# JoakimHaurum/TokenReduction

Measured on AMD Instinct MI355X. Metric: images/sec DeiT-S Top-K keep_rate=0.7 forward (aggregate over n_gpus; per-GPU = value/n_gpus), higher is better.
Workload: dtype bf16; 1 GPU; topk_small_patch16_224 keep_rate=0.7 reduction_loc=3,6,9 batch=256/GPU 224x224 eval forward (BASELINE.json configs[1]); global_batch=256, parallelism=dp1

## Files before the change

tokenreduction_amd/csrc/tr_mlp_fused.hip:

```cpp
#include "tr_common.h"

__device__ unsigned long long tr_mlp_clock_probe[3];

namespace {

#ifdef TR_ABLATE_NO_MFMA
#define MF_MFMA(a, b, c) ([&] { asm volatile("" ::"v"(a), "v"(b)); return c; }())
#else
#define MF_MFMA(a, b, c) __builtin_amdgcn_mfma_f32_16x16x32_bf16(a, b, c, 0, 0, 0)
#endif
__device__ __forceinline__ float mf_gelu1(float x) {
  constexpr float L2E = 1.44269504088896340736f;
  constexpr float C1 = -1.59501577f * L2E, C3 = -7.40112920e-02f * L2E, C5 = 7.03033576e-04f * L2E;
  const float xc = __builtin_amdgcn_fmed3f(x, -8.0f, 8.0f);
  const float x2 = xc * xc;
  float p = __builtin_fmaf(x2, C5, C3);
  p = __builtin_fmaf(p, x2, C1);
  const float z = p * xc;
  const float e = __builtin_amdgcn_exp2f(z) + 1.0f;
  return x * __builtin_amdgcn_rcpf(e);
}
#if defined(TR_ABLATE_NO_GELU)
__device__ __forceinline__ f32x2 mf_gelu2(f32x2 v) { return v; }
#elif defined(MF_GELU_PACKED)
// ... 3 lines not shown
  float a = mf_gelu1(v[0]), b = mf_gelu1(v[1]);
  asm volatile("" : "+v"(a), "+v"(b));
  return f32x2{a, b};
}
#endif

typedef __attribute__((ext_vector_type(4))) unsigned u32x4;
typedef __attribute__((ext_vector_type(2))) unsigned u32x2;

#ifdef MF_ABL_NO_XSTORE
#define MF_XSTORE(x) asm volatile("" ::"v"(v))
#else
#define MF_XSTORE(x) x
#endif
#ifdef MF_ABL_NO_NSTORE
#define MF_NSTORE(x) do { } while (0)
#else
#define MF_NSTORE(x) x
#endif
#ifdef TR_DIAG_STAMPS
#define MF_STAMP(k) ts_[k] = __builtin_amdgcn_s_memtime()
#define MF_STAMP_DECL unsigned long long ts_[4] = {0, 0, 0, 0}
#define MF_STAMP_DUMP(role, step)                                                                                                     \
  do {                                                                                                                                \
    if (bid == 8 && pr == 0 && lane == 0 && (step) < 64) {                                                                            \
      unsigned long long* st_ = reinterpret_cast<unsigned long long*>(reinterpret_cast<unsigned char*>(outp) + out_bytes) + ((role) * 64 + (step)) * 4; \
      st_[0] = ts_[0]; st_[1] = ts_[1]; st_[2] = ts_[2]; st_[3] = ts_[3];                                                             \
    }                                                                                                                                 \
  } while (0)
#define MF_ESTAMP(k) es_[k] = __builtin_amdgcn_s_memtime()
#define MF_ESTAMP_DECL unsigned long long es_[8] = {0, 0, 0, 0, 0, 0, 0, 0}
#define MF_ESTAMP_DUMP                                                                                                                \
  do {                                                                                                                                \
    if (bid == 8 && pr == 0 && lane == 0) {                                                                                           \
      unsigned long long* st_ = reinterpret_cast<unsigned long long*>(reinterpret_cast<unsigned char*>(outp) + out_bytes) + 60 * 4;   \
      for (int k_ = 0; k_ < 8; ++k_) st_[k_] = es_[k_];                                                                               \
    }                                                                                                                                 \
  } while (0)
#define MF_CLOCK_BEGIN const unsigned long long ck0_ = __builtin_amdgcn_s_memtime(), rt0_ = __builtin_amdgcn_s_memrealtime()
#define MF_CLOCK_END                                                                                                                  \
  do {                                                                                                                                \
    if (bid == 8 && tid == 0) {                                                                                                       \
      unsigned long long* st_ = reinterpret_cast<unsigned long long*>(reinterpret_cast<unsigned char*>(outp) + out_bytes) + 512;      \
      st_[0] = __builtin_amdgcn_s_memtime() - ck0_;                                                                                   \
      st_[1] = __builtin_amdgcn_s_memrealtime() - rt0_;                                                                               \
    }                                                                                                                                 \
  } while (0)
#elif defined(TR_DIAG_CLOCK)
#define MF_CLOCK_BEGIN const unsigned long long ck0_ = __builtin_amdgcn_s_memtime(), rt0_ = __builtin_amdgcn_s_memrealtime()
#define MF_CLOCK_END                                                                                                                  \
  do {                                                                                                                                \
    if (bid == 8 && tid == 0) {                                                                                                       \
      atomicAdd(&tr_mlp_clock_probe[0], __builtin_amdgcn_s_memtime() - ck0_);                                                         \
      atomicAdd(&tr_mlp_clock_probe[1], __builtin_amdgcn_s_memrealtime() - rt0_);                                                     \
      atomicAdd(&tr_mlp_clock_probe[2], 1ull);                                                                                        \
    }                                                                                                                                 \
  } while (0)
#define MF_STAMP(k) do { } while (0)
#define MF_STAMP_DECL do { } while (0)
#define MF_STAMP_DUMP(role, step) do { } while (0)
#define MF_ESTAMP(k) do { } while (0)
#define MF_ESTAMP_DECL do { } while (0)
#define MF_ESTAMP_DUMP do { } while (0)
#else
#define MF_CLOCK_BEGIN do { } while (0)
#define MF_CLOCK_END do { } while (0)
#define MF_STAMP(k) do { } while (0)
#define MF_STAMP_DECL do { } while (0)
#define MF_STAMP_DUMP(role, step) do { } while (0)
#define MF_ESTAMP(k) do { } while (0)
#define MF_ESTAMP_DECL do { } while (0)
#define MF_ESTAMP_DUMP do { } while (0)
#endif

constexpr int MF_D = 384;
constexpr int MF_KS = MF_D / 32;
constexpr int MF_NI = MF_D / 16;
constexpr int MF_W1FR = 2 * MF_KS;
constexpr int MF_FR = MF_W1FR + MF_NI;
constexpr int MF_ENTRY = MF_FR * 1024;
constexpr int MF_NSLOT = 3;
constexpr int MF_HBUF = 2048;
constexpr int MF_LDS = MF_NSLOT * MF_ENTRY + 4 * 2 * MF_HBUF;
constexpr int MF_ROWS = 128;
#ifndef MF_PQ
#define MF_PQ 0
#endif
#ifndef MF_DMA_BURST
#define MF_DMA_SPREAD 1
#endif
constexpr int MF_PPW = (MF_PQ + 3) / 4;
[[maybe_unused]] constexpr int MF_CPW = (12 - MF_PQ + 4) / 5;

__device__ __forceinline__ void mf_piece(const unsigned char* sbase, unsigned voff, unsigned lds_dst) {
#ifndef TR_ABLATE_NO_DMA
  asm volatile(
      "s_mov_b32 m0, %[ld]\n\t"
      "s_nop 0\n\t"
      "global_load_lds_dwordx4 %[o], %[b]"
      :
      : [o] "v"(voff), [b] "s"(sbase), [ld] "s"(lds_dst)
      : "memory", "m0");
#endif
}

template <int IMM>
__device__ __forceinline__ bf16x8 mf_load_x(const uint16_t* sbase, unsigned voff) {
  bf16x8 v;
  asm volatile("global_load_dwordx4 %0, %1, %2 offset:%3" : "=v"(v) : "v"(voff), "s"(sbase), "i"(IMM) : "memory");
  return v;
}
template <int IMM>
__device__ __forceinline__ void mf_reload_x(bf16x8& v, const uint16_t* sbase, unsigned voff) {
  asm volatile("global_load_dwordx4 %0, %1, %2 offset:%3" : "+v"(v) : "v"(voff), "s"(sbase), "i"(IMM) : "memory");
}
template <int IMM>
__device__ __forceinline__ f32x4 mf_load_f4(const float* sbase, unsigned voff) {
  f32x4 v;
  asm volatile("global_load_dwordx4 %0, %1, %2 offset:%3" : "=v"(v) : "v"(voff), "s"(sbase), "i"(IMM) : "memory");
  return v;
}

#define MF_TIE_X(x)                                                                                                                   \
  "+v"(x[0]), "+v"(x[1]), "+v"(x[2]), "+v"(x[3]), "+v"(x[4]), "+v"(x[5]), "+v"(x[6]), "+v"(x[7]), "+v"(x[8]), "+v"(x[9]), "+v"(x[10]), \
      "+v"(x[11])

__global__ __launch_bounds__(256) void mlp_pack_kernel(const uint16_t* __restrict__ W1, const uint16_t* __restrict__ W2, const float* __restrict__ b2,
                                                       u32x4* __restrict__ pk, int D, int Hd) {
  const int ks_n = D / 32, ni = D / 16, fr = 2 * ks_n + ni;
  const int g = blockIdx.x * 4 + (threadIdx.x >> 6);
  const int lane = threadIdx.x & 63;
  const int s = g / fr, f = g % fr;
  if (s >= Hd / 32) {
    const int e = g - (Hd / 32) * fr;
    if (e < 2 * ni) pk[(size_t)g * 64 + lane] = *reinterpret_cast<const u32x4*>(b2 + 16 * (e >> 1) + 4 * (lane >> 4));
    return;
  }
  const int r = lane & 15, q = lane >> 4;
  const uint16_t* src;
  if (f < 2 * ks_n) {
#ifdef MF_P32
    const int rho = lane & 31, kq = lane >> 5;
    const int hh = 8 * (((rho >> 2) & 1) + 2 * (rho >> 4)) + 4 * ((rho >> 3) & 1) + (rho & 3);
    src = W1 + (size_t)(32 * s + hh) * D + 16 * f + 8 * kq;
#else
    const int t2 = f / ks_n, ks = f % ks_n;
    src = W1 + (size_t)(32 * s + 8 * (r >> 2) + 4 * t2 + (r & 3)) * D + 32 * ks + 8 * q;
#endif
  } else {
    const int i = f - 2 * ks_n;
    src = W2 + (size_t)(16 * i + r) * Hd + 32 * s + 8 * q;
  }
  pk[(size_t)g * 64 + lane] = *reinterpret_cast<const u32x4*>(src);
}

struct MfSeq {
  int head_len, head_blk;
  int full0, fstride, nfull;
  int tail_s0, tail_blk;
};
struct MfCur {
  int seg, s;
};
__device__ __forceinline__ MfCur mf_first(const MfSeq& q, int NS) {
  if (q.head_len > 0) return MfCur{-1, 0};
  if (q.nfull > 0) return MfCur{0, 0};
// ... 17 lines not shown
constexpr unsigned MF_SK_ERR_MAGIC = 0x4d46534bu;

struct MfResid {
  float* x;
  const float* b2;
  const float* g;
  const float* b;
  float eps;
};

struct MfNorm {
  const float* x;
  const uint16_t* d;
  const float* g;
  const float* b;
  float eps;
};

template <bool RL, bool NP>
__global__ __launch_bounds__(512, 2) void mlp_fused_kernel(const uint16_t* __restrict__ xn, const unsigned char* __restrict__ pk,
                                                           const float* __restrict__ b1,
                                                           uint16_t* __restrict__ outp, unsigned char* __restrict__ scratch, int M, int NS,
                                                           unsigned out_bytes, int poll_max, int cset, const MfResid rl, const MfNorm nm) {
  __shared__ __attribute__((aligned(16))) unsigned char smem[MF_LDS];
  const int tid = threadIdx.x, lane = tid & 63;
  const int wave = __builtin_amdgcn_readfirstlane(tid >> 6);
  const int pr = wave & 3;
#ifdef MF_XCD_RANGES
  const int G = gridDim.x;
  const int bid = (G % 8 == 0 && G > 8) ? ((int)blockIdx.x & 7) * (G >> 3) + ((int)blockIdx.x >> 3) : (int)blockIdx.x;
#else
  const int G = gridDim.x, bid = blockIdx.x;
#endif
  const int nblk = (M + MF_ROWS - 1) / MF_ROWS;
  if (bid >= nblk) return;
  MfSeq q;
  int T;
  const bool streamk = scratch != nullptr && nblk > G;
  if (!streamk) {
    q = MfSeq{0, 0, bid, G, (nblk - bid + G - 1) / G, NS, 0};
    T = q.nfull * NS;
  } else {
    const long long U = (long long)nblk * NS;
    const int u0 = (int)(U * bid / G), u1 = (int)(U * (bid + 1) / G);
    const int b_first = u0 / NS, s0 = u0 - b_first * NS;
    const int b_end = u1 / NS, s1 = u1 - b_end * NS;
    const int f0 = s0 > 0 ? b_first + 1 : b_first;
    q = MfSeq{s1, b_end, f0, 1, b_end - f0, s0 > 0 ? s0 : NS, b_first};
    T = u1 - u0;
  }
  q.head_len = __builtin_amdgcn_readfirstlane(q.head_len); q.head_blk = __builtin_amdgcn_readfirstlane(q.head_blk);
  q.full0 = __builtin_amdgcn_readfirstlane(q.full0); q.fstride = __builtin_amdgcn_readfirstlane(q.fstride);
  q.nfull = __builtin_amdgcn_readfirstlane(q.nfull); q.tail_s0 = __builtin_amdgcn_readfirstlane(q.tail_s0);
  q.tail_blk = __builtin_amdgcn_readfirstlane(q.tail_blk);
  T = __builtin_amdgcn_readfirstlane(T);
  const unsigned lds0 = (unsigned)(uintptr_t)(__attribute__((address_space(3))) unsigned char*)smem;
  const unsigned lane16 = (unsigned)lane * 16u;
  const int frow = lane & 15, fq = lane >> 4;
  unsigned char* const hb = smem + MF_NSLOT * MF_ENTRY + pr * (2 * MF_HBUF);

  MfCur ld_cur = mf_first(q, NS);
  int ld_e = 0, ld_w1 = ld_cur.s, ld_w2 = ld_cur.s, ld_w2n = ld_cur.s, ld_slot = 0;
  auto issue_piece_q = [&](int q) __attribute__((always_inline)) {
    const int f = (wave < 4 ? 0 : 4 * MF_PQ) + pr + 4 * q;
    const int step = (f < MF_W1FR) ? ld_w1 : ld_w2;
    mf_piece(pk + (size_t)step * MF_ENTRY + f * 1024, lane16, lds0 + ld_slot * MF_ENTRY + f * 1024);
  };
  auto issue_all = [&]() __attribute__((always_inline)) {
    if (wave < 4) {
#pragma unroll
      for (int q = 0; q < MF_PQ; ++q) issue_piece_q(q);
    } else {
#pragma unroll
      for (int q = 0; q < 12 - MF_PQ; ++q) issue_piece_q(q);
    }
  };
  auto advance_entry = [&]() __attribute__((always_inline)) {
    ++ld_e;
    ld_w2 = ld_w2n;
    ld_w2n = ld_w1;
    ld_cur = mf_next(q, ld_cur, NS);
    ld_w1 = ld_cur.s;
    ld_slot = (ld_slot + 1 == MF_NSLOT) ? 0 : ld_slot + 1;
  };

#ifdef MF_P32
  if (wave < 4) {
    typedef __attribute__((ext_vector_type(16))) float f32x16;
    const int tc = lane & 31, hg = lane >> 5;
    bf16x8 xk[2 * MF_KS];
    auto x_offset = [&](int blk) __attribute__((always_inline)) {
      const int m = blk * MF_ROWS + pr * 32 + tc;
      return ((unsigned)min(m, M - 1) * MF_D + 8u * hg) * 2u;
    };
    {
      const unsigned xo = x_offset(mf_block(q, mf_first(q, NS)));
#define MF_LX(ks) xk[ks] = mf_load_x<(ks) * 32>(xn, xo)
      MF_LX(0); MF_LX(1); MF_LX(2); MF_LX(3); MF_LX(4); MF_LX(5); MF_LX(6); MF_LX(7); MF_LX(8); MF_LX(9); MF_LX(10); MF_LX(11);
      MF_LX(12); MF_LX(13); MF_LX(14); MF_LX(15); MF_LX(16); MF_LX(17); MF_LX(18); MF_LX(19); MF_LX(20); MF_LX(21); MF_LX(22); MF_LX(23);
#undef MF_LX
    }
    const unsigned boff = (unsigned)hg * 32u;
    f32x4 bn0, bn1, bn2, bn3;
    bn0 = mf_load_f4<0>(b1 + 32 * mf_first(q, NS).s, boff);
    bn1 = mf_load_f4<16>(b1 + 32 * mf_first(q, NS).s, boff);
    bn2 = mf_load_f4<64>(b1 + 32 * mf_first(q, NS).s, boff);
    bn3 = mf_load_f4<80>(b1 + 32 * mf_first(q, NS).s, boff);
    issue_all();
    advance_entry();
    issue_all();
    advance_entry();
#define MF_TIE_XK(lo) "+v"(xk[lo]), "+v"(xk[lo + 1]), "+v"(xk[lo + 2]), "+v"(xk[lo + 3]), "+v"(xk[lo + 4]), "+v"(xk[lo + 5]), "+v"(xk[lo + 6]), "+v"(xk[lo + 7]), "+v"(xk[lo + 8]), "+v"(xk[lo + 9]), "+v"(xk[lo + 10]), "+v"(xk[lo + 11])
    asm volatile("s_waitcnt vmcnt(0)" : "+v"(bn0), "+v"(bn1), "+v"(bn2), "+v"(bn3), MF_TIE_XK(0), MF_TIE_XK(12)::"memory");
    __builtin_amdgcn_s_barrier();
    asm volatile("" ::: "memory");

    int t = 0, cslot = 0;
    f32x4 p0, p1, p2, p3;
    p0 = p1 = p2 = p3 = f32x4{0.f, 0.f, 0.f, 0.f};
    asm volatile("" : "+v"(p0), "+v"(p1), "+v"(p2), "+v"(p3));
    bf16x8 wA[4], wB[4];
#define MF_READW(buf, base, k)                                                     \
  buf[0] = *reinterpret_cast<const bf16x8*>((base) + (4 * (k)) * 1024);            \
  buf[1] = *reinterpret_cast<const bf16x8*>((base) + (4 * (k) + 1) * 1024);        \
  buf[2] = *reinterpret_cast<const bf16x8*>((base) + (4 * (k) + 2) * 1024);        \
  buf[3] = *reinterpret_cast<const bf16x8*>((base) + (4 * (k) + 3) * 1024)
    MF_READW(wA, smem + lane16, 0);
    MF_CLOCK_BEGIN;
    const unsigned hdst = (unsigned)((tc >> 4) * 1024 + ((tc & 15) + 16 * hg) * 16);
    auto p_step = [&](int sn, const bool last, int next_blk) __attribute__((always_inline)) {
      const unsigned char* slot = smem + cslot * MF_ENTRY + lane16;
      const int nslot = (cslot + 1 == MF_NSLOT) ? 0 : cslot + 1;
      const unsigned char* slot_next = smem + nslot * MF_ENTRY + lane16;
      MF_STAMP_DECL;
      MF_STAMP(0);
      f32x16 a;
#pragma unroll
      for (int e = 0; e < 4; ++e) { a[e] = bn0[e]; a[4 + e] = bn1[e]; a[8 + e] = bn2[e]; a[12 + e] = bn3[e]; }
      u32x4 h0 = {0u, 0u, 0u, 0u}, h1 = {0u, 0u, 0u, 0u};
      unsigned xo = 0;
      const bool reload = last && next_blk >= 0;
      if (reload) xo = x_offset(next_blk);
#define MF_GELU_SLICE(k)                                                                                  \
  do {                                                                                                    \
    if ((k) == 0) { const f32x2 g0 = mf_gelu2(f32x2{p0[0], p0[1]}), g1 = mf_gelu2(f32x2{p0[2], p0[3]}); h0[0] = pack_bf16x2(g0[0], g0[1]); h0[1] = pack_bf16x2(g1[0], g1[1]); asm volatile("" : "+v"(h0[0]), "+v"(h0[1])); } \
    if ((k) == 1) { const f32x2 g0 = mf_gelu2(f32x2{p1[0], p1[1]}), g1 = mf_gelu2(f32x2{p1[2], p1[3]}); h0[2] = pack_bf16x2(g0[0], g0[1]); h0[3] = pack_bf16x2(g1[0], g1[1]); asm volatile("" : "+v"(h0[2]), "+v"(h0[3])); } \
    if ((k) == 2) { const f32x2 g0 = mf_gelu2(f32x2{p2[0], p2[1]}), g1 = mf_gelu2(f32x2{p2[2], p2[3]}); h1[0] = pack_bf16x2(g0[0], g0[1]); h1[1] = pack_bf16x2(g1[0], g1[1]); asm volatile("" : "+v"(h1[0]), "+v"(h1[1])); } \
    if ((k) == 3) { const f32x2 g0 = mf_gelu2(f32x2{p3[0], p3[1]}), g1 = mf_gelu2(f32x2{p3[2], p3[3]}); h1[2] = pack_bf16x2(g0[0], g0[1]); h1[3] = pack_bf16x2(g1[0], g1[1]); asm volatile("" : "+v"(h1[2]), "+v"(h1[3])); } \
    if ((k) == 4) {                                                                                       \
      unsigned char* dst = hb + ((t - 1) & 1) * MF_HBUF + hdst;                                           \
      *reinterpret_cast<u32x4*>(dst) = h0;                                                                \
      *reinterpret_cast<u32x4*>(dst + 512) = h1;                                                          \
    }                                                                                                     \
  } while (0)
#define MF_PMFMA(cur, k)                                                                                           \
  do {                                                                                                             \
    a = __builtin_amdgcn_mfma_f32_32x32x16_bf16(cur[0], xk[4 * (k)], a, 0, 0, 0);                                  \
    a = __builtin_amdgcn_mfma_f32_32x32x16_bf16(cur[1], xk[4 * (k) + 1], a, 0, 0, 0);                              \
    a = __builtin_amdgcn_mfma_f32_32x32x16_bf16(cur[2], xk[4 * (k) + 2], a, 0, 0, 0);                              \
    a = __builtin_amdgcn_mfma_f32_32x32x16_bf16(cur[3], xk[4 * (k) + 3], a, 0, 0, 0);                              \
  } while (0)
#define MF_RX(ks) mf_reload_x<(ks) * 32>(xk[ks], xn, xo)
#define MF_PWIN(cur, nxt, k)                                                                    \
  do {                                                                                          \
    MF_READW(nxt, slot, (k) + 1);                                                               \
    __builtin_amdgcn_sched_barrier(0);                                                          \
// ... 6 lines not shown
      bn2 = mf_load_f4<64>(b1 + 32 * sn, boff);                                                 \
      bn3 = mf_load_f4<80>(b1 + 32 * sn, boff);                                                 \
    }                                                                                           \
    if (reload) { MF_RX(4 * (k)); MF_RX(4 * (k) + 1); MF_RX(4 * (k) + 2); MF_RX(4 * (k) + 3); } \
  } while (0)
      MF_PWIN(wA, wB, 0);
      MF_PWIN(wB, wA, 1);
      MF_PWIN(wA, wB, 2);
      MF_PWIN(wB, wA, 3);
      MF_PWIN(wA, wB, 4);
      if (ld_e <= T + 1) advance_entry();
      MF_STAMP(1);
      if (last) asm volatile("s_waitcnt vmcnt(0)" ::: "memory");
      asm volatile("s_waitcnt vmcnt(0)" : "+v"(bn0), "+v"(bn1), "+v"(bn2), "+v"(bn3), MF_TIE_XK(0), MF_TIE_XK(12)::"memory");
      asm volatile("s_waitcnt lgkmcnt(0)" ::: "memory");
      MF_STAMP(2);
      __builtin_amdgcn_s_barrier();
      asm volatile("" ::: "memory");
      MF_STAMP(3);
      MF_READW(wA, slot_next, 0);
      __builtin_amdgcn_sched_barrier(0);
      MF_PMFMA(wB, 5);
      __builtin_amdgcn_sched_barrier(0);
      if (reload) { MF_RX(20); MF_RX(21); MF_RX(22); MF_RX(23); }
#undef MF_PWIN
#undef MF_GELU_SLICE
#pragma unroll
      for (int e = 0; e < 4; ++e) { p0[e] = a[e]; p1[e] = a[4 + e]; p2[e] = a[8 + e]; p3[e] = a[12 + e]; }
      MF_STAMP_DUMP(0, t);
      ++t;
      cslot = nslot;
    };
    {
      MfCur cur = mf_first(q, NS);
      for (int tt = 0; tt < T; ++tt) {
        const MfCur nxt = mf_next(q, cur, NS);
        int last = __builtin_amdgcn_readfirstlane(mf_last_of_segment(q, cur, NS) ? 1 : 0);
        asm volatile("" : "+s"(last));
        p_step(nxt.s, last != 0, (last && tt + 1 < T) ? mf_block(q, nxt) : -1);
        cur = nxt;
      }
    }
    {
      const f32x2 g0 = mf_gelu2(f32x2{p0[0], p0[1]}), g1 = mf_gelu2(f32x2{p0[2], p0[3]});
      const f32x2 g2 = mf_gelu2(f32x2{p1[0], p1[1]}), g3 = mf_gelu2(f32x2{p1[2], p1[3]});
      const u32x4 h0 = {pack_bf16x2(g0[0], g0[1]), pack_bf16x2(g1[0], g1[1]), pack_bf16x2(g2[0], g2[1]), pack_bf16x2(g3[0], g3[1])};
      const f32x2 g4 = mf_gelu2(f32x2{p2[0], p2[1]}), g5 = mf_gelu2(f32x2{p2[2], p2[3]});
      const f32x2 g6 = mf_gelu2(f32x2{p3[0], p3[1]}), g7 = mf_gelu2(f32x2{p3[2], p3[3]});
      const u32x4 h1 = {pack_bf16x2(g4[0], g4[1]), pack_bf16x2(g5[0], g5[1]), pack_bf16x2(g6[0], g6[1]), pack_bf16x2(g7[0], g7[1])};
      unsigned char* dst = hb + ((t - 1) & 1) * MF_HBUF + hdst;
      *reinterpret_cast<u32x4*>(dst) = h0;
      *reinterpret_cast<u32x4*>(dst + 512) = h1;
      asm volatile("s_waitcnt vmcnt(0) lgkmcnt(0)" ::: "memory");
      __builtin_amdgcn_s_barrier();
    }
#undef MF_PMFMA
#undef MF_READW
#undef MF_RX
#undef MF_TIE_XK
    if constexpr (RL) __builtin_amdgcn_s_barrier();
    MF_CLOCK_END;
    return;
  }
#else
  if (wave < 4) {
#ifdef MF_PRIO_P
    __builtin_amdgcn_s_setprio(MF_PRIO_P);
#endif
    bf16x8 x0[MF_KS], x1[MF_KS];
    f32x4 bn0, bn1;
    const unsigned boff = (unsigned)fq * 32u;
    auto x_offsets = [&](int blk, unsigned& o0, unsigned& o1) __attribute__((always_inline)) {
      const int m = blk * MF_ROWS + pr * 32 + frow;
      o0 = ((unsigned)min(m, M - 1) * MF_D + 8u * fq) * 2u;
      o1 = ((unsigned)min(m + 16, M - 1) * MF_D + 8u * fq) * 2u;
    };
#define MF_LOAD_X(ks)                          \
  x0[ks] = mf_load_x<(ks) * 64>(xn, xo0);      \
  x1[ks] = mf_load_x<(ks) * 64>(xn, xo1)
#define MF_RELOAD_X(ks)                        \
  mf_reload_x<(ks) * 64>(x0[ks], xn, xo0);     \
  mf_reload_x<(ks) * 64>(x1[ks], xn, xo1)
    auto ln_fill = [&](int blk) __attribute__((always_inline)) {
#pragma unroll
      for (int j = 0; j < 2; ++j) {
        const int m = min(blk * MF_ROWS + pr * 32 + frow + 16 * j, M - 1);
        const float* xr = nm.x + (size_t)m * MF_D + 8 * fq;
        const uint16_t* dr = nm.d + (size_t)m * MF_D + 8 * fq;
        f32x4 v[MF_KS][2];
        u32x4 dq[2][4];
#pragma unroll
        for (int i = 0; i < 4; ++i) dq[0][i] = *reinterpret_cast<const u32x4*>(dr + 32 * i);
#pragma unroll
        for (int ks = 0; ks < MF_KS; ++ks) {
          v[ks][0] = *reinterpret_cast<const f32x4*>(xr + 32 * ks);
          v[ks][1] = *reinterpret_cast<const f32x4*>(xr + 32 * ks + 4);
        }
        __builtin_amdgcn_sched_barrier(0);
#pragma unroll
        for (int c = 0; c < 3; ++c) {
          if (c + 1 < 3) {
#pragma unroll
            for (int i = 0; i < 4; ++i) dq[(c + 1) & 1][i] = *reinterpret_cast<const u32x4*>(dr + 32 * (4 * (c + 1) + i));
          }
          __builtin_amdgcn_sched_barrier(0);
#pragma unroll
          for (int i = 0; i < 4; ++i) {
            const u32x4 dd = dq[c & 1][i];
            const int ks = 4 * c + i;
#pragma unroll
            for (int h = 0; h < 2; ++h) {
              v[ks][h][0] += __uint_as_float(dd[2 * h] << 16); v[ks][h][1] += __uint_as_float(dd[2 * h] & 0xffff0000u);
              v[ks][h][2] += __uint_as_float(dd[2 * h + 1] << 16); v[ks][h][3] += __uint_as_float(dd[2 * h + 1] & 0xffff0000u);
            }
          }
          __builtin_amdgcn_sched_barrier(0);
        }
        float sp[4][2];
#pragma unroll
        for (int ks = 0; ks < MF_KS; ++ks)
#pragma unroll
          for (int h = 0; h < 2; ++h) {
            const float t = (v[ks][h][0] + v[ks][h][1]) + (v[ks][h][2] + v[ks][h][3]);
            sp[ks & 3][h] = (ks < 4 ? 0.f : sp[ks & 3][h]) + t;
          }
        float c0 = (sp[0][0] + sp[2][0]) + (sp[1][0] + sp[3][0]), c1 = (sp[0][1] + sp[2][1]) + (sp[1][1] + sp[3][1]);
        c0 += __shfl_xor(c0, 32); c1 += __shfl_xor(c1, 32);
        c0 += __shfl_xor(c0, 16); c1 += __shfl_xor(c1, 16);
        const float mean = (c0 + c1) / (float)MF_D;
        __builtin_amdgcn_sched_barrier(0);
#pragma unroll
        for (int ks = 0; ks < MF_KS; ++ks)
#pragma unroll
          for (int h = 0; h < 2; ++h) {
            f32x4 t = v[ks][h];
            t[0] -= mean; t[1] -= mean; t[2] -= mean; t[3] -= mean;
            v[ks][h] = t;
            const float u = __builtin_fmaf(t[0], t[0], t[1] * t[1]) + __builtin_fmaf(t[2], t[2], t[3] * t[3]);
            sp[ks & 3][h] = (ks < 4 ? 0.f : sp[ks & 3][h]) + u;
          }
        c0 = (sp[0][0] + sp[2][0]) + (sp[1][0] + sp[3][0]); c1 = (sp[0][1] + sp[2][1]) + (sp[1][1] + sp[3][1]);
        c0 += __shfl_xor(c0, 32); c1 += __shfl_xor(c1, 32);
        c0 += __shfl_xor(c0, 16); c1 += __shfl_xor(c1, 16);
        const float rstd = rsqrtf((c0 + c1) / (float)MF_D + nm.eps);
        const float* gr = nm.g + 8 * fq;
        const float* br = nm.b + 8 * fq;
        f32x4 gb[2][4];
        gb[0][0] = *reinterpret_cast<const f32x4*>(gr); gb[0][1] = *reinterpret_cast<const f32x4*>(gr + 4);
        gb[0][2] = *reinterpret_cast<const f32x4*>(br); gb[0][3] = *reinterpret_cast<const f32x4*>(br + 4);
        __builtin_amdgcn_sched_barrier(0);
#pragma unroll
        for (int ks = 0; ks < MF_KS; ++ks) {
          if (ks + 1 < MF_KS) {
            gb[(ks + 1) & 1][0] = *reinterpret_cast<const f32x4*>(gr + 32 * (ks + 1)); gb[(ks + 1) & 1][1] = *reinterpret_cast<const f32x4*>(gr + 32 * (ks + 1) + 4);
            gb[(ks + 1) & 1][2] = *reinterpret_cast<const f32x4*>(br + 32 * (ks + 1)); gb[(ks + 1) & 1][3] = *reinterpret_cast<const f32x4*>(br + 32 * (ks + 1) + 4);
          }
          __builtin_amdgcn_sched_barrier(0);
          u32x4 o;
#pragma unroll
          for (int h = 0; h < 2; ++h) {
            const f32x4 gg = gb[ks & 1][h], bb = gb[ks & 1][2 + h];
            const f32x4 t = v[ks][h];
            o[2 * h] = pack_bf16x2(__builtin_fmaf(rstd * t[0], gg[0], bb[0]), __builtin_fmaf(rstd * t[1], gg[1], bb[1]));
            o[2 * h + 1] = pack_bf16x2(__builtin_fmaf(rstd * t[2], gg[2], bb[2]), __builtin_fmaf(rstd * t[3], gg[3], bb[3]));
          }
          if (j == 0) x0[ks] = __builtin_bit_cast(bf16x8, o);
          else x1[ks] = __builtin_bit_cast(bf16x8, o);
          __builtin_amdgcn_sched_barrier(0);
        }
      }
    };
    if constexpr (NP) {
      ln_fill(mf_block(q, mf_first(q, NS)));
    } else {
      unsigned xo0, xo1;
      x_offsets(mf_block(q, mf_first(q, NS)), xo0, xo1);
      MF_LOAD_X(0); MF_LOAD_X(1); MF_LOAD_X(2); MF_LOAD_X(3); MF_LOAD_X(4); MF_LOAD_X(5);
      MF_LOAD_X(6); MF_LOAD_X(7); MF_LOAD_X(8); MF_LOAD_X(9); MF_LOAD_X(10); MF_LOAD_X(11);
    }
    bn0 = mf_load_f4<0>(b1 + 32 * mf_first(q, NS).s, boff);
    bn1 = mf_load_f4<16>(b1 + 32 * mf_first(q, NS).s, boff);
    issue_all();
    advance_entry();
    issue_all();
    advance_entry();
    asm volatile("s_waitcnt vmcnt(0)" : "+v"(bn0), "+v"(bn1), MF_TIE_X(x0), MF_TIE_X(x1)::"memory");
    __builtin_amdgcn_s_barrier();
    asm volatile("" ::: "memory");

    int t = 0, cslot = 0;
    f32x4 p00, p01, p10, p11;
    p00 = p01 = p10 = p11 = f32x4{0.f, 0.f, 0.f, 0.f};
    asm volatile("" : "+v"(p00), "+v"(p01), "+v"(p10), "+v"(p11));
    bf16x8 wA[4], wB[4];
#define MF_READW(buf, base, k)                                                                  \
  buf[0] = *reinterpret_cast<const bf16x8*>((base) + (2 * (k)) * 1024);                        \
  buf[1] = *reinterpret_cast<const bf16x8*>((base) + (MF_KS + 2 * (k)) * 1024);                \
  buf[2] = *reinterpret_cast<const bf16x8*>((base) + (2 * (k) + 1) * 1024);                    \
  buf[3] = *reinterpret_cast<const bf16x8*>((base) + (MF_KS + 2 * (k) + 1) * 1024)
    MF_READW(wA, smem + lane16, 0);
    MF_CLOCK_BEGIN;
    auto p_step = [&](int sn, const bool last, int next_blk) __attribute__((always_inline)) {
      const unsigned char* slot = smem + cslot * MF_ENTRY + lane16;
      const int nslot = (cslot + 1 == MF_NSLOT) ? 0 : cslot + 1;
      const unsigned char* slot_next = smem + nslot * MF_ENTRY + lane16;
      MF_STAMP_DECL;
      MF_STAMP(0);
      f32x4 a00 = bn0, a01 = bn0, a10 = bn1, a11 = bn1;
      u32x4 h0 = {0u, 0u, 0u, 0u}, h1 = {0u, 0u, 0u, 0u};
      unsigned xo0 = 0, xo1 = 0;
      const bool reload = last && next_blk >= 0;
      if (reload) x_offsets(next_blk, xo0, xo1);
      const bool dma = ld_e <= T + 1;
#define MF_GELU_SLICE(k)                                                                                  \
  do {                                                                                                    \
    if ((k) == 0) { const f32x2 g0 = mf_gelu2(f32x2{p00[0], p00[1]}), g1 = mf_gelu2(f32x2{p00[2], p00[3]}); h0[0] = pack_bf16x2(g0[0], g0[1]); h0[1] = pack_bf16x2(g1[0], g1[1]); asm volatile("" : "+v"(h0[0]), "+v"(h0[1])); } \
    if ((k) == 1) { const f32x2 g0 = mf_gelu2(f32x2{p10[0], p10[1]}), g1 = mf_gelu2(f32x2{p10[2], p10[3]}); h0[2] = pack_bf16x2(g0[0], g0[1]); h0[3] = pack_bf16x2(g1[0], g1[1]); asm volatile("" : "+v"(h0[2]), "+v"(h0[3])); } \
    if ((k) == 2) { const f32x2 g0 = mf_gelu2(f32x2{p01[0], p01[1]}), g1 = mf_gelu2(f32x2{p01[2], p01[3]}); h1[0] = pack_bf16x2(g0[0], g0[1]); h1[1] = pack_bf16x2(g1[0], g1[1]); asm volatile("" : "+v"(h1[0]), "+v"(h1[1])); } \
    if ((k) == 3) { const f32x2 g0 = mf_gelu2(f32x2{p11[0], p11[1]}), g1 = mf_gelu2(f32x2{p11[2], p11[3]}); h1[2] = pack_bf16x2(g0[0], g0[1]); h1[3] = pack_bf16x2(g1[0], g1[1]); asm volatile("" : "+v"(h1[2]), "+v"(h1[3])); } \
    if ((k) == 4) {                                                                                       \
      unsigned char* dst = hb + ((t - 1) & 1) * MF_HBUF + lane16;                                         \
      *reinterpret_cast<u32x4*>(dst) = h0;                                                                \
      *reinterpret_cast<u32x4*>(dst + 1024) = h1;                                                         \
    }                                                                                                     \
  } while (0)
#define MF_PMFMA(cur, k)                                                                        \
  do {                                                                                          \
    a00 = MF_MFMA(cur[0], x0[2 * (k)], a00);                                                    \
    a01 = MF_MFMA(cur[0], x1[2 * (k)], a01);                                                    \
    a10 = MF_MFMA(cur[1], x0[2 * (k)], a10);                                                    \
    a11 = MF_MFMA(cur[1], x1[2 * (k)], a11);                                                    \
    a00 = MF_MFMA(cur[2], x0[2 * (k) + 1], a00);                                                \
    a01 = MF_MFMA(cur[2], x1[2 * (k) + 1], a01);                                                \
    a10 = MF_MFMA(cur[3], x0[2 * (k) + 1], a10);                                                \
    a11 = MF_MFMA(cur[3], x1[2 * (k) + 1], a11);                                                \
  } while (0)
#define MF_PWIN(cur, nxt, k)                                                                    \
  do {                                                                                          \
    MF_READW(nxt, slot, (k) + 1);                                                               \
    __builtin_amdgcn_sched_barrier(0);                                                          \
    MF_PMFMA(cur, k);                                                                           \
    MF_GELU_SLICE(k);                                                                           \
    __builtin_amdgcn_sched_barrier(0);                                                          \
    if ((k) == 0) {                                                                             \
       \
      bn0 = mf_load_f4<0>(b1 + 32 * sn, boff);                                                  \
      bn1 = mf_load_f4<16>(b1 + 32 * sn, boff);                                                 \
    }                                                                                           \
    if ((k) >= 1 && dma) {                                                                      \
      _Pragma("unroll") for (int q_ = MF_PPW * ((k) - 1); q_ < MF_PPW * (k); ++q_)              \
        if (q_ < MF_PQ) issue_piece_q(q_);                                                      \
    }                                                                                           \
    if (!NP && reload) { MF_RELOAD_X(2 * (k)); MF_RELOAD_X(2 * (k) + 1); }                      \
  } while (0)
      MF_PWIN(wA, wB, 0);
      MF_PWIN(wB, wA, 1);
      MF_PWIN(wA, wB, 2);
      MF_PWIN(wB, wA, 3);
      MF_PWIN(wA, wB, 4);
      if (dma) advance_entry();
      MF_STAMP(1);
      if (last) asm volatile("s_waitcnt vmcnt(0)" ::: "memory");
      asm volatile("s_waitcnt vmcnt(%26)" : "+v"(bn0), "+v"(bn1), MF_TIE_X(x0), MF_TIE_X(x1) : "n"(MF_PQ) : "memory");
      asm volatile("s_waitcnt lgkmcnt(0)" ::: "memory");
      MF_STAMP(2);
      __builtin_amdgcn_s_barrier();
      asm volatile("" ::: "memory");
      MF_STAMP(3);
      MF_READW(wA, slot_next, 0);
      __builtin_amdgcn_sched_barrier(0);
      MF_PMFMA(wB, 5);
      __builtin_amdgcn_sched_barrier(0);
      if constexpr (NP) {
        if (reload) {
          ln_fill(next_blk);
          MF_READW(wA, slot_next, 0);
        }
      } else {
        if (reload) { MF_RELOAD_X(10); MF_RELOAD_X(11); }
      }
#undef MF_PWIN
#undef MF_GELU_SLICE
      p00 = a00; p01 = a01; p10 = a10; p11 = a11;
      MF_STAMP_DUMP(0, t);
      ++t;
      cslot = nslot;
    };
    {
      MfCur cur = mf_first(q, NS);
      for (int tt = 0; tt < T; ++tt) {
        const MfCur nxt = mf_next(q, cur, NS);
        int last = __builtin_amdgcn_readfirstlane(mf_last_of_segment(q, cur, NS) ? 1 : 0);
        asm volatile("" : "+s"(last));
        p_step(nxt.s, last != 0, (last && tt + 1 < T) ? mf_block(q, nxt) : -1);
        cur = nxt;
      }
    }
    {
      const f32x2 g0 = mf_gelu2(f32x2{p00[0], p00[1]}), g1 = mf_gelu2(f32x2{p00[2], p00[3]});
      const f32x2 g2 = mf_gelu2(f32x2{p10[0], p10[1]}), g3 = mf_gelu2(f32x2{p10[2], p10[3]});
      const u32x4 h0 = {pack_bf16x2(g0[0], g0[1]), pack_bf16x2(g1[0], g1[1]), pack_bf16x2(g2[0], g2[1]), pack_bf16x2(g3[0], g3[1])};
      const f32x2 g4 = mf_gelu2(f32x2{p01[0], p01[1]}), g5 = mf_gelu2(f32x2{p01[2], p01[3]});
      const f32x2 g6 = mf_gelu2(f32x2{p11[0], p11[1]}), g7 = mf_gelu2(f32x2{p11[2], p11[3]});
      const u32x4 h1 = {pack_bf16x2(g4[0], g4[1]), pack_bf16x2(g5[0], g5[1]), pack_bf16x2(g6[0], g6[1]), pack_bf16x2(g7[0], g7[1])};
      unsigned char* dst = hb + ((t - 1) & 1) * MF_HBUF + lane16;
      *reinterpret_cast<u32x4*>(dst) = h0;
      *reinterpret_cast<u32x4*>(dst + 1024) = h1;
      asm volatile("s_waitcnt vmcnt(0) lgkmcnt(0)" ::: "memory");
      __builtin_amdgcn_s_barrier();
    }
#undef MF_PMFMA
#undef MF_READW
#undef MF_LOAD_X
#undef MF_RELOAD_X
    if constexpr (RL) __builtin_amdgcn_s_barrier();
    MF_CLOCK_END;
    return;
  }

#endif
#ifdef MF_PRIO_C
  __builtin_amdgcn_s_setprio(MF_PRIO_C);
#endif
  const __amdgpu_buffer_rsrc_t orsrc = __builtin_amdgcn_make_buffer_rsrc(outp, 0, (int)out_bytes, 0x00020000);
  const unsigned char* const bias_img = pk + (size_t)NS * MF_ENTRY;
  f32x4 acc[MF_NI][2];
  const __amdgpu_buffer_rsrc_t xrsrc = __builtin_amdgcn_make_buffer_rsrc(RL ? reinterpret_cast<unsigned char*>(rl.x) : const_cast<unsigned char*>(bias_img), 0,
                                                                         RL ? (int)(2u * out_bytes) : MF_NI * 2 * 1024, 0x00020000);
  auto x_row_off = [&](int blk) __attribute__((always_inline)) { return ((unsigned)(blk * MF_ROWS + pr * 32 + frow) * MF_D + 4u * fq) * 4u; };
  if constexpr (RL) {
    const unsigned vo = x_row_off(mf_block(q, mf_first(q, NS)));
#pragma unroll
    for (int i = 0; i < MF_NI; ++i)
#pragma unroll
      for (int j = 0; j < 2; ++j)
        acc[i][j] = __builtin_bit_cast(f32x4, __builtin_amdgcn_raw_buffer_load_b128(xrsrc, vo + (unsigned)(j * 16 * MF_D * 4), i * 64, 0));
  } else {
#pragma unroll
    for (int i = 0; i < MF_NI; ++i)
#pragma unroll
      for (int j = 0; j < 2; ++j)
        acc[i][j] = __builtin_bit_cast(f32x4, __builtin_amdgcn_raw_buffer_load_b128(xrsrc, lane16 + (unsigned)((i * 2 + j) * 1024), 0, 0));
  }
  issue_all();
  advance_entry();
  issue_all();
  advance_entry();
  asm volatile("s_waitcnt vmcnt(0)" ::: "memory");
  __builtin_amdgcn_s_barrier();
  asm volatile("" ::: "memory");

  int t = 0, cslot = 0;
  bf16x8 wA[4], wB[4];
  bf16x8 h0, h1;
#define MF_READW(buf, base, k)                                                     \
  buf[0] = *reinterpret_cast<const bf16x8*>((base) + (4 * (k)) * 1024);            \
  buf[1] = *reinterpret_cast<const bf16x8*>((base) + (4 * (k) + 1) * 1024);        \
  buf[2] = *reinterpret_cast<const bf16x8*>((base) + (4 * (k) + 2) * 1024);        \
  buf[3] = *reinterpret_cast<const bf16x8*>((base) + (4 * (k) + 3) * 1024)
  for (; t < 2; ++t) {
    if (ld_e <= T + 1) {
      issue_all();
      advance_entry();
    }
    cslot = (cslot + 1 == MF_NSLOT) ? 0 : cslot + 1;
    asm volatile("s_waitcnt vmcnt(%0)" ::"n"(12 - MF_PQ) : "memory");
    __builtin_amdgcn_s_barrier();
    asm volatile("" ::: "memory");
  }
  {
    const unsigned char* hsrc = hb + (t & 1) * MF_HBUF + lane16;
    h0 = *reinterpret_cast<const bf16x8*>(hsrc);
    h1 = *reinterpret_cast<const bf16x8*>(hsrc + 1024);
    MF_READW(wA, smem + cslot * MF_ENTRY + MF_W1FR * 1024 + lane16, 0);
  }
  const __amdgpu_buffer_rsrc_t sk_out = __builtin_amdgcn_make_buffer_rsrc(scratch + (size_t)bid * MF_SK_SLOT, 0, MF_SK_SLOT, 0x00020000);
  unsigned char* const sk_cnt0 = scratch + (size_t)G * MF_SK_SLOT + MF_SK_ERR + (size_t)cset * G * MF_SK_CNT;
  unsigned* const sk_cnt_out = reinterpret_cast<unsigned*>(sk_cnt0 + (size_t)bid * MF_SK_CNT);
  unsigned* const sk_cnt_in = reinterpret_cast<unsigned*>(sk_cnt0 + (size_t)(bid > 0 ? bid - 1 : 0) * MF_SK_CNT);
  bool publish_pending = false;
  auto c_step = [&](const int fin, const bool load_next, int blk, int blk_next) __attribute__((always_inline)) {
    const bool epi = fin == 1;
    const unsigned char* slot = smem + cslot * MF_ENTRY + MF_W1FR * 1024 + lane16;
    const int nslot = (cslot + 1 == MF_NSLOT) ? 0 : cslot + 1;
    const unsigned char* slot_next = smem + nslot * MF_ENTRY + MF_W1FR * 1024 + lane16;
    MF_STAMP_DECL;
    MF_STAMP(0);
    const bool dma = ld_e <= T + 1;
#define MF_CMFMA(cur, k)                                                                                           \
  _Pragma("unroll") for (int ii = 0; ii < 4; ++ii) {                                                               \
    acc[4 * (k) + ii][0] = MF_MFMA(cur[ii], h0, acc[4 * (k) + ii][0]);                                             \
    acc[4 * (k) + ii][1] = MF_MFMA(cur[ii], h1, acc[4 * (k) + ii][1]);                                             \
  }
#if defined(MF_DMA_SPREAD)
#define MF_CWIN(cur, nxt, k)                                                                                       \
  do {                                                                                                             \
    MF_READW(nxt, slot, (k) + 1);                                                                                  \
    __builtin_amdgcn_sched_barrier(0);                                                                             \
    _Pragma("unroll") for (int ii = 0; ii < 4; ++ii) {                                                             \
      acc[4 * (k) + ii][0] = MF_MFMA(cur[ii], h0, acc[4 * (k) + ii][0]);                                           \
      acc[4 * (k) + ii][1] = MF_MFMA(cur[ii], h1, acc[4 * (k) + ii][1]);                                           \
      __builtin_amdgcn_sched_barrier(0);                                                                           \
      const int hk_ = 4 * (k) + ii;                                                                                \
      if (((hk_ + 1) * (12 - MF_PQ)) / 20 > (hk_ * (12 - MF_PQ)) / 20) {                                           \
        if (dma) issue_piece_q((hk_ * (12 - MF_PQ)) / 20);                                                         \
      }                                                                                                            \
    }                                                                                                              \
  } while (0)
#else
#define MF_CWIN(cur, nxt, k)                                                                                       \
  do {                                                                                                             \
    MF_READW(nxt, slot, (k) + 1);                                                                                  \
    __builtin_amdgcn_sched_barrier(0);                                                                             \
    MF_CMFMA(cur, k);                                                                                              \
    __builtin_amdgcn_sched_barrier(0);                                                                             \
    if (dma) {                                                                                                     \
      _Pragma("unroll") for (int q_ = MF_CPW * (k); q_ < MF_CPW * ((k) + 1); ++q_)                                 \
        if (q_ < 12 - MF_PQ) issue_piece_q(q_);                                                                    \
    }                                                                                                              \
  } while (0)
#endif
    MF_CWIN(wA, wB, 0);
    MF_CWIN(wB, wA, 1);
    MF_CWIN(wA, wB, 2);
    MF_CWIN(wB, wA, 3);
    MF_CWIN(wA, wB, 4);
#undef MF_CWIN
    if (dma) advance_entry();
    MF_STAMP(1);
    if (t <= T) {
// ... 442 lines not shown
```

Baseline: 105,900 images/s.

## Split first-block LayerNorm between producer and consumer waves via LDS hand-over

For the fused-norm prologue, producer waves now normalize only the first 16-row group. Consumer waves normalize the second group and hand it over through a free ring slot in LDS. Gamma and beta are DMA'd once into LDS for this first block, and weight-slot prefetch is issued before or inside the norm so it overlaps the LN loads. This shortens the serial prologue on the producer waves, at the cost of an extra barrier, LDS traffic and tighter coupling between wave roles.

Result: faster. 107,600 images/s (median of 6 runs) (+1.6%).

```diff
diff --git a/tokenreduction_amd/csrc/tr_mlp_fused.hip b/tokenreduction_amd/csrc/tr_mlp_fused.hip
--- a/tokenreduction_amd/csrc/tr_mlp_fused.hip
+++ b/tokenreduction_amd/csrc/tr_mlp_fused.hip
@@ -109,6 +109,12 @@
 constexpr int MF_NSLOT = 3;
 constexpr int MF_HBUF = 2048;
 constexpr int MF_LDS = MF_NSLOT * MF_ENTRY + 4 * 2 * MF_HBUF;
+constexpr int MF_LNX = 2 * MF_ENTRY;
+static_assert(4 * MF_KS * 1024 <= MF_ENTRY, "the hand-over rows of the four pairs fit one ring slot");
+constexpr int MF_LNP = MF_NSLOT * MF_ENTRY;
+static_assert(2 * MF_D * 4 <= 4 * 2 * MF_HBUF, "the norm's two vectors fit the hidden buffers");
+template <bool V>
+struct MfFlag { static constexpr bool value = V; };
 constexpr int MF_ROWS = 128;
 #ifndef MF_PQ
 #define MF_PQ 0
@@ -292,6 +298,104 @@
     ld_cur = mf_next(q, ld_cur, NS);
     ld_w1 = ld_cur.s;
     ld_slot = (ld_slot + 1 == MF_NSLOT) ? 0 : ld_slot + 1;
+  };
+
+  [[maybe_unused]] auto ln_group = [&](int blk, const int j, auto first, auto&& after_loads, auto&& emit) __attribute__((always_inline)) {
+    constexpr bool FIRST = decltype(first)::value;
+    const int m = min(blk * MF_ROWS + pr * 32 + frow + 16 * j, M - 1);
+    const float* xr = nm.x + (size_t)m * MF_D + 8 * fq;
+    const uint16_t* dr = nm.d + (size_t)m * MF_D + 8 * fq;
+    f32x4 v[MF_KS][2];
+    u32x4 dq[2][4];
+    if constexpr (FIRST) {
+      mf_piece(reinterpret_cast<const unsigned char*>(nm.g), lane16, lds0 + MF_LNP);
+      mf_piece(reinterpret_cast<const unsigned char*>(nm.b), lane16, lds0 + MF_LNP + MF_D * 4);
+      if (lane < 32) {
+        mf_piece(reinterpret_cast<const unsigned char*>(nm.g) + 1024, lane16, lds0 + MF_LNP + 1024);
+        mf_piece(reinterpret_cast<const unsigned char*>(nm.b) + 1024, lane16, lds0 + MF_LNP + MF_D * 4 + 1024);
+      }
+    }
+#pragma unroll
+    for (int i = 0; i < 4; ++i) dq[0][i] = *reinterpret_cast<const u32x4*>(dr + 32 * i);
+#pragma unroll
+    for (int ks = 0; ks < MF_KS; ++ks) {
+      v[ks][0] = *reinterpret_cast<const f32x4*>(xr + 32 * ks);
+      v[ks][1] = *reinterpret_cast<const f32x4*>(xr + 32 * ks + 4);
+    }
+    __builtin_amdgcn_sched_barrier(0);
+    after_loads();
+    __builtin_amdgcn_sched_barrier(0);
+#pragma unroll
+    for (int c = 0; c < 3; ++c) {
+      if (c + 1 < 3) {
+#pragma unroll
+        for (int i = 0; i < 4; ++i) dq[(c + 1) & 1][i] = *reinterpret_cast<const u32x4*>(dr + 32 * (4 * (c + 1) + i));
+      }
+      __builtin_amdgcn_sched_barrier(0);
+#pragma unroll
+      for (int i = 0; i < 4; ++i) {
+        const u32x4 dd = dq[c & 1][i];
+        const int ks = 4 * c + i;
+#pragma unroll
+        for (int h = 0; h < 2; ++h) {
+          v[ks][h][0] += __uint_as_float(dd[2 * h] << 16); v[ks][h][1] += __uint_as_float(dd[2 * h] & 0xffff0000u);
+          v[ks][h][2] += __uint_as_float(dd[2 * h + 1] << 16); v[ks][h][3] += __uint_as_float(dd[2 * h + 1] & 0xffff0000u);
+        }
+      }
+      __builtin_amdgcn_sched_barrier(0);
+    }
+    float sp[4][2];
+#pragma unroll
+    for (int ks = 0; ks < MF_KS; ++ks)
+#pragma unroll
+      for (int h = 0; h < 2; ++h) {
+        const float t = (v[ks][h][0] + v[ks][h][1]) + (v[ks][h][2] + v[ks][h][3]);
+        sp[ks & 3][h] = (ks < 4 ? 0.f : sp[ks & 3][h]) + t;
+      }
+    float c0 = (sp[0][0] + sp[2][0]) + (sp[1][0] + sp[3][0]), c1 = (sp[0][1] + sp[2][1]) + (sp[1][1] + sp[3][1]);
+    c0 += __shfl_xor(c0, 32); c1 += __shfl_xor(c1, 32);
+    c0 += __shfl_xor(c0, 16); c1 += __shfl_xor(c1, 16);
+    const float mean = (c0 + c1) / (float)MF_D;
+    __builtin_amdgcn_sched_barrier(0);
+#pragma unroll
+    for (int ks = 0; ks < MF_KS; ++ks)
+#pragma unroll
+      for (int h = 0; h < 2; ++h) {
+        f32x4 t = v[ks][h];
+        t[0] -= mean; t[1] -= mean; t[2] -= mean; t[3] -= mean;
+        v[ks][h] = t;
+        const float u = __builtin_fmaf(t[0], t[0], t[1] * t[1]) + __builtin_fmaf(t[2], t[2], t[3] * t[3]);
+        sp[ks & 3][h] = (ks < 4 ? 0.f : sp[ks & 3][h]) + u;
+      }
+    c0 = (sp[0][0] + sp[2][0]) + (sp[1][0] + sp[3][0]); c1 = (sp[0][1] + sp[2][1]) + (sp[1][1] + sp[3][1]);
+    c0 += __shfl_xor(c0, 32); c1 += __shfl_xor(c1, 32);
+    c0 += __shfl_xor(c0, 16); c1 += __shfl_xor(c1, 16);
+    const float rstd = rsqrtf((c0 + c1) / (float)MF_D + nm.eps);
+    if constexpr (FIRST) asm volatile("s_waitcnt vmcnt(0)" ::: "memory");
+    const float* gr = FIRST ? reinterpret_cast<const float*>(smem + MF_LNP) + 8 * fq : nm.g + 8 * fq;
+    const float* br = FIRST ? reinterpret_cast<const float*>(smem + MF_LNP) + MF_D + 8 * fq : nm.b + 8 * fq;
+    f32x4 gb[2][4];
+    gb[0][0] = *reinterpret_cast<const f32x4*>(gr); gb[0][1] = *reinterpret_cast<const f32x4*>(gr + 4);
+    gb[0][2] = *reinterpret_cast<const f32x4*>(br); gb[0][3] = *reinterpret_cast<const f32x4*>(br + 4);
+    __builtin_amdgcn_sched_barrier(0);
+#pragma unroll
+    for (int ks = 0; ks < MF_KS; ++ks) {
+      if (ks + 1 < MF_KS) {
+        gb[(ks + 1) & 1][0] = *reinterpret_cast<const f32x4*>(gr + 32 * (ks + 1)); gb[(ks + 1) & 1][1] = *reinterpret_cast<const f32x4*>(gr + 32 * (ks + 1) + 4);
+        gb[(ks + 1) & 1][2] = *reinterpret_cast<const f32x4*>(br + 32 * (ks + 1)); gb[(ks + 1) & 1][3] = *reinterpret_cast<const f32x4*>(br + 32 * (ks + 1) + 4);
+      }
+      __builtin_amdgcn_sched_barrier(0);
+      u32x4 o;
+#pragma unroll
+      for (int h = 0; h < 2; ++h) {
+        const f32x4 gg = gb[ks & 1][h], bb = gb[ks & 1][2 + h];
+        const f32x4 t = v[ks][h];
+        o[2 * h] = pack_bf16x2(__builtin_fmaf(rstd * t[0], gg[0], bb[0]), __builtin_fmaf(rstd * t[1], gg[1], bb[1]));
+        o[2 * h + 1] = pack_bf16x2(__builtin_fmaf(rstd * t[2], gg[2], bb[2]), __builtin_fmaf(rstd * t[3], gg[3], bb[3]));
+      }
+      emit(ks, o);
+      __builtin_amdgcn_sched_barrier(0);
+    }
   };
 
 #ifdef MF_P32
@@ -464,96 +568,20 @@
   mf_reload_x<(ks) * 64>(x0[ks], xn, xo0);     \
   mf_reload_x<(ks) * 64>(x1[ks], xn, xo1)
     auto ln_fill = [&](int blk) __attribute__((always_inline)) {
-#pragma unroll
-      for (int j = 0; j < 2; ++j) {
-        const int m = min(blk * MF_ROWS + pr * 32 + frow + 16 * j, M - 1);
-        const float* xr = nm.x + (size_t)m * MF_D + 8 * fq;
-        const uint16_t* dr = nm.d + (size_t)m * MF_D + 8 * fq;
-        f32x4 v[MF_KS][2];
-        u32x4 dq[2][4];
-#pragma unroll
-        for (int i = 0; i < 4; ++i) dq[0][i] = *reinterpret_cast<const u32x4*>(dr + 32 * i);
-#pragma unroll
-        for (int ks = 0; ks < MF_KS; ++ks) {
-          v[ks][0] = *reinterpret_cast<const f32x4*>(xr + 32 * ks);
-          v[ks][1] = *reinterpret_cast<const f32x4*>(xr + 32 * ks + 4);
-        }
-        __builtin_amdgcn_sched_barrier(0);
-#pragma unroll
-        for (int c = 0; c < 3; ++c) {
-          if (c + 1 < 3) {
-#pragma unroll
-            for (int i = 0; i < 4; ++i) dq[(c + 1) & 1][i] = *reinterpret_cast<const u32x4*>(dr + 32 * (4 * (c + 1) + i));
-          }
-          __builtin_amdgcn_sched_barrier(0);
-#pragma unroll
-          for (int i = 0; i < 4; ++i) {
-            const u32x4 dd = dq[c & 1][i];
-            const int ks = 4 * c + i;
-#pragma unroll
-            for (int h = 0; h < 2; ++h) {
-              v[ks][h][0] += __uint_as_float(dd[2 * h] << 16); v[ks][h][1] += __uint_as_float(dd[2 * h] & 0xffff0000u);
-              v[ks][h][2] += __uint_as_float(dd[2 * h + 1] << 16); v[ks][h][3] += __uint_as_float(dd[2 * h + 1] & 0xffff0000u);
-            }
-          }
-          __builtin_amdgcn_sched_barrier(0);
-        }
-        float sp[4][2];
-#pragma unroll
-        for (int ks = 0; ks < MF_KS; ++ks)
-#pragma unroll
-          for (int h = 0; h < 2; ++h) {
-            const float t = (v[ks][h][0] + v[ks][h][1]) + (v[ks][h][2] + v[ks][h][3]);
-            sp[ks & 3][h] = (ks < 4 ? 0.f : sp[ks & 3][h]) + t;
-          }
-        float c0 = (sp[0][0] + sp[2][0]) + (sp[1][0] + sp[3][0]), c1 = (sp[0][1] + sp[2][1]) + (sp[1][1] + sp[3][1]);
-        c0 += __shfl_xor(c0, 32); c1 += __shfl_xor(c1, 32);
-        c0 += __shfl_xor(c0, 16); c1 += __shfl_xor(c1, 16);
-        const float mean = (c0 + c1) / (float)MF_D;
-        __builtin_amdgcn_sched_barrier(0);
-#pragma unroll
-        for (int ks = 0; ks < MF_KS; ++ks)
-#pragma unroll
-          for (int h = 0; h < 2; ++h) {
-            f32x4 t = v[ks][h];
-            t[0] -= mean; t[1] -= mean; t[2] -= mean; t[3] -= mean;
-            v[ks][h] = t;
-            const float u = __builtin_fmaf(t[0], t[0], t[1] * t[1]) + __builtin_fmaf(t[2], t[2], t[3] * t[3]);
-            sp[ks & 3][h] = (ks < 4 ? 0.f : sp[ks & 3][h]) + u;
-          }
-        c0 = (sp[0][0] + sp[2][0]) + (sp[1][0] + sp[3][0]); c1 = (sp[0][1] + sp[2][1]) + (sp[1][1] + sp[3][1]);
-        c0 += __shfl_xor(c0, 32); c1 += __shfl_xor(c1, 32);
-        c0 += __shfl_xor(c0, 16); c1 += __shfl_xor(c1, 16);
-        const float rstd = rsqrtf((c0 + c1) / (float)MF_D + nm.eps);
-        const float* gr = nm.g + 8 * fq;
-        const float* br = nm.b + 8 * fq;
-        f32x4 gb[2][4];
-        gb[0][0] = *reinterpret_cast<const f32x4*>(gr); gb[0][1] = *reinterpret_cast<const f32x4*>(gr + 4);
-        gb[0][2] = *reinterpret_cast<const f32x4*>(br); gb[0][3] = *reinterpret_cast<const f32x4*>(br + 4);
-        __builtin_amdgcn_sched_barrier(0);
-#pragma unroll
-        for (int ks = 0; ks < MF_KS; ++ks) {
-          if (ks + 1 < MF_KS) {
-            gb[(ks + 1) & 1][0] = *reinterpret_cast<const f32x4*>(gr + 32 * (ks + 1)); gb[(ks + 1) & 1][1] = *reinterpret_cast<const f32x4*>(gr + 32 * (ks + 1) + 4);
-            gb[(ks + 1) & 1][2] = *reinterpret_cast<const f32x4*>(br + 32 * (ks + 1)); gb[(ks + 1) & 1][3] = *reinterpret_cast<const f32x4*>(br + 32 * (ks + 1) + 4);
-          }
-          __builtin_amdgcn_sched_barrier(0);
-          u32x4 o;
-#pragma unroll
-          for (int h = 0; h < 2; ++h) {
-            const f32x4 gg = gb[ks & 1][h], bb = gb[ks & 1][2 + h];
-            const f32x4 t = v[ks][h];
-            o[2 * h] = pack_bf16x2(__builtin_fmaf(rstd * t[0], gg[0], bb[0]), __builtin_fmaf(rstd * t[1], gg[1], bb[1]));
-            o[2 * h + 1] = pack_bf16x2(__builtin_fmaf(rstd * t[2], gg[2], bb[2]), __builtin_fmaf(rstd * t[3], gg[3], bb[3]));
-          }
-          if (j == 0) x0[ks] = __builtin_bit_cast(bf16x8, o);
-          else x1[ks] = __builtin_bit_cast(bf16x8, o);
-          __builtin_amdgcn_sched_barrier(0);
-        }
-      }
+      ln_group(blk, 0, MfFlag<false>{}, [] {}, [&](int ks, const u32x4 o) __attribute__((always_inline)) { x0[ks] = __builtin_bit_cast(bf16x8, o); });
+      ln_group(blk, 1, MfFlag<false>{}, [] {}, [&](int ks, const u32x4 o) __attribute__((always_inline)) { x1[ks] = __builtin_bit_cast(bf16x8, o); });
     };
     if constexpr (NP) {
-      ln_fill(mf_block(q, mf_first(q, NS)));
+      issue_all();
+      advance_entry();
+      issue_all();
+      advance_entry();
+      ln_group(mf_block(q, mf_first(q, NS)), 0, MfFlag<true>{}, [] {}, [&](int ks, const u32x4 o) __attribute__((always_inline)) { x0[ks] = __builtin_bit_cast(bf16x8, o); });
+      __builtin_amdgcn_s_barrier();
+      asm volatile("" ::: "memory");
+      const unsigned char* hx = smem + MF_LNX + pr * (MF_KS * 1024) + lane16;
+#pragma unroll
+      for (int ks = 0; ks < MF_KS; ++ks) x1[ks] = *reinterpret_cast<const bf16x8*>(hx + ks * 1024);
     } else {
       unsigned xo0, xo1;
       x_offsets(mf_block(q, mf_first(q, NS)), xo0, xo1);
@@ -562,10 +590,12 @@
     }
     bn0 = mf_load_f4<0>(b1 + 32 * mf_first(q, NS).s, boff);
     bn1 = mf_load_f4<16>(b1 + 32 * mf_first(q, NS).s, boff);
-    issue_all();
-    advance_entry();
-    issue_all();
-    advance_entry();
+    if constexpr (!NP) {
+      issue_all();
+      advance_entry();
+      issue_all();
+      advance_entry();
+    }
     asm volatile("s_waitcnt vmcnt(0)" : "+v"(bn0), "+v"(bn1), MF_TIE_X(x0), MF_TIE_X(x1)::"memory");
     __builtin_amdgcn_s_barrier();
     asm volatile("" ::: "memory");
@@ -710,6 +740,17 @@
   const __amdgpu_buffer_rsrc_t xrsrc = __builtin_amdgcn_make_buffer_rsrc(RL ? reinterpret_cast<unsigned char*>(rl.x) : const_cast<unsigned char*>(bias_img), 0,
                                                                          RL ? (int)(2u * out_bytes) : MF_NI * 2 * 1024, 0x00020000);
   auto x_row_off = [&](int blk) __attribute__((always_inline)) { return ((unsigned)(blk * MF_ROWS + pr * 32 + frow) * MF_D + 4u * fq) * 4u; };
+  if constexpr (NP) {
+    unsigned char* const hx = smem + MF_LNX + pr * (MF_KS * 1024) + lane16;
+    ln_group(mf_block(q, mf_first(q, NS)), 1, MfFlag<true>{},
+             [&]() __attribute__((always_inline)) {
+               issue_all();
+               advance_entry();
+               issue_all();
+               advance_entry();
+             },
+             [&](int ks, const u32x4 o) __attribute__((always_inline)) { *reinterpret_cast<u32x4*>(hx + ks * 1024) = o; });
+  }
   if constexpr (RL) {
     const unsigned vo = x_row_off(mf_block(q, mf_first(q, NS)));
 #pragma unroll
@@ -724,10 +765,16 @@
       for (int j = 0; j < 2; ++j)
         acc[i][j] = __builtin_bit_cast(f32x4, __builtin_amdgcn_raw_buffer_load_b128(xrsrc, lane16 + (unsigned)((i * 2 + j) * 1024), 0, 0));
   }
-  issue_all();
-  advance_entry();
-  issue_all();
-  advance_entry();
+  if constexpr (NP) {
+    asm volatile("s_waitcnt lgkmcnt(0)" ::: "memory");
+    __builtin_amdgcn_s_barrier();
+    asm volatile("" ::: "memory");
+  } else {
+    issue_all();
+    advance_entry();
+    issue_all();
+    advance_entry();
+  }
   asm volatile("s_waitcnt vmcnt(0)" ::: "memory");
   __builtin_amdgcn_s_barrier();
   asm volatile("" ::: "memory");
```
